# BaguaSys/bagua

Measured on AMD Instinct MI355X. Metric: images/sec (whole node), VGG16 GradientAllReduce vs ByteGrad at 1/2/4/8 MI355X, higher is better.
Workload: dtype bf16; 1 GPU; model=vgg16, algorithm=gradient_allreduce, backend=bagua, global_batch=32, image_size=224, parallelism=dp1

## Files before the change

bagua_amd/models/vgg.py:

```python

from typing import List, Union

import torch
import torch.nn as nn
import torch.nn.functional as F

from ..ops import conv_epilogue

_CFGS = {
    "A": [64, "M", 128, "M", 256, 256, "M", 512, 512, "M", 512, 512, "M"],
    "B": [64, 64, "M", 128, 128, "M", 256, 256, "M", 512, 512, "M",
          512, 512, "M"],
    "D": [64, 64, "M", 128, 128, "M", 256, 256, 256, "M", 512, 512, 512,
          "M", 512, 512, 512, "M"],
    "E": [64, 64, "M", 128, 128, "M", 256, 256, 256, 256, "M",
          512, 512, 512, 512, "M", 512, 512, 512, 512, "M"],
}


class VGG(nn.Module):
    def __init__(self, cfg: List[Union[int, str]], num_classes: int = 1000,
                 batch_norm: bool = False, dropout: float = 0.5):
        super().__init__()
        layers: List[nn.Module] = []
        in_ch = 3
        for v in cfg:
            if v == "M":
                layers.append(nn.MaxPool2d(kernel_size=2, stride=2))
            else:
                layers.append(nn.Conv2d(in_ch, v, kernel_size=3, padding=1))
                if batch_norm:
                    layers.append(nn.BatchNorm2d(v))
                layers.append(nn.ReLU(inplace=True))
                in_ch = v
        self.features = nn.Sequential(*layers)
        self.avgpool = nn.AdaptiveAvgPool2d((7, 7))
        self.classifier = nn.Sequential(
            nn.Linear(512 * 7 * 7, 4096),
            nn.ReLU(True),
            nn.Dropout(p=dropout),
            nn.Linear(4096, 4096),
            nn.ReLU(True),
            nn.Dropout(p=dropout),
            nn.Linear(4096, num_classes),
        )

    torch_bias_grad = False

    def _features(self, x: torch.Tensor) -> torch.Tensor:
        if _has_hooks(self.features):
            return self.features(x)
        mods = list(self.features)
        i = 0
        while i < len(mods):
            m = mods[i]
            step = _fusable(mods, i)
            if step:
                pool = step == 3 and conv_epilogue.conv_eligible(x, m, True)
                if pool or conv_epilogue.conv_eligible(x, m, False):
                    x = F.conv2d(x, m.weight, None, m.stride, m.padding,
                                 m.dilation, m.groups)
                    x = conv_epilogue.conv_bias_relu(
                        x, m.bias, pool, self.torch_bias_grad)
                    i += 3 if pool else 2
                    continue
            x = m(x)
            i += 1
        return x

    def forward(self, x: torch.Tensor) -> torch.Tensor:
        x = self._features(x)
        x = self.avgpool(x)
        x = torch.flatten(x, 1)
        return self.classifier(x)


def _has_hooks(m: nn.Module) -> bool:
    return bool(m._forward_hooks or m._forward_pre_hooks
                or m._backward_hooks or m._backward_pre_hooks)


def _fusable(mods, i) -> int:
    if i + 1 >= len(mods):
        return 0
    conv, relu = mods[i], mods[i + 1]
    if type(conv) is not nn.Conv2d or type(relu) is not nn.ReLU:
        return 0
    if _has_hooks(conv) or _has_hooks(relu):
        return 0
    if i + 2 < len(mods):
        p = mods[i + 2]
        if (type(p) is nn.MaxPool2d and not _has_hooks(p)
                and p.kernel_size in (2, (2, 2)) and p.stride in (2, (2, 2))
                and p.padding in (0, (0, 0)) and p.dilation in (1, (1, 1))
                and not p.ceil_mode and not p.return_indices):
            return 3
    return 2


def vgg11(num_classes=1000, batch_norm=False):
    return VGG(_CFGS["A"], num_classes, batch_norm)


def vgg13(num_classes=1000, batch_norm=False):
    return VGG(_CFGS["B"], num_classes, batch_norm)


def vgg16(num_classes=1000, batch_norm=False):
    return VGG(_CFGS["D"], num_classes, batch_norm)


def vgg19(num_classes=1000, batch_norm=False):
    return VGG(_CFGS["E"], num_classes, batch_norm)
```

bagua_amd/ops/csrc/core.cpp:

```cpp

#include <torch/extension.h>

#include <hip/hip_runtime_api.h>
#include <rccl/rccl.h>

#include <c10/hip/HIPCachingAllocator.h>
#include <c10/hip/HIPStream.h>

#include <chrono>
#include <cmath>
#include <condition_variable>
#include <cstring>
#include <memory>
#include <mutex>
#include <optional>
#include <stdexcept>
#include <string>
#include <thread>
#include <vector>

extern "C" {
void bagua_ew_launch(int op, int dtype, void* x, const void* y, float f,
                     size_t n, hipStream_t stream);
void bagua_async_avg_launch(int dtype, void* x, const void* reduced,
                            const void* x_copy, float nranks, size_t n,
                            hipStream_t stream);
void bagua_reduce_chunk_launch(int dtype, void* x, int num_chunks,
                               int target_chunk, int average, size_t chunk,
                               hipStream_t stream);
void bagua_compress_launch(int dtype, const void* x, uint8_t* out,
                           uint32_t* scratch, uint32_t* partials,
                           size_t chunk, size_t chunk_stride,
                           int num_chunks_total, int chunk_begin,
                           int chunk_count, hipStream_t stream);
void bagua_decompress_launch(int dtype, const uint8_t* in, void* x,
                             size_t chunk, size_t chunk_stride,
                             int chunk_begin, int chunk_count,
                             hipStream_t stream);
void bagua_dequant_reduce_launch(int dtype, const uint8_t* in, void* x,
                                 size_t chunk, size_t chunk_stride,
                                 int num_chunks, int target_chunk,
                                 int average, hipStream_t stream);
void bagua_fused_sgd_launch(float* p, const float* g, float* m, float lr,
                            float momentum, float dampening,
                            float weight_decay, int nesterov,
                            int momentum_initialized, size_t n,
                            hipStream_t stream);
void bagua_fused_adam_launch(float* p, const float* g, float* m, float* v,
                             float lr, float beta1, float beta2,
                             float one_minus_beta1, float one_minus_beta2,
                             float eps, float weight_decay, int adamw,
                             float bc1, float bc2, size_t n,
                             hipStream_t stream);
void bagua_fused_sgd_mixed_launch(void* p, const void* g, float* master,
                                  float* m, float lr, float momentum,
                                  float dampening, float weight_decay,
                                  int nesterov, int momentum_initialized,
                                  size_t n, hipStream_t stream);
void bagua_fused_sgd_segments_launch(float* p, float* m, float lr,
                                     float momentum, float dampening,
                                     float weight_decay, int nesterov,
                                     int momentum_initialized,
                                     const void* const* grads,
                                     const size_t* begins,
                                     const size_t* numels, size_t count,
                                     hipStream_t stream);
void bagua_fused_sgd_mixed_segments_launch(
    void* p, float* master, float* m, float lr, float momentum,
    float dampening, float weight_decay, int nesterov,
    int momentum_initialized, const void* const* grads, const size_t* begins,
    const size_t* numels, size_t count, hipStream_t stream);
void bagua_fused_adam_segments_launch(
    float* p, float* m, float* v, float lr, float beta1, float beta2,
    float one_minus_beta1, float one_minus_beta2, float eps,
    float weight_decay, int adamw, float bc1, float bc2,
    const void* const* grads, const size_t* begins, const size_t* numels,
    size_t count, hipStream_t stream);
}

extern "C" {
size_t bagua_moe_assign_workspace(int S, int E);
void bagua_moe_assign_slots_launch(const int* expert, int S, int E,
                                   int capacity, const int* base, int* hist,
                                   int* slot, int* counts, int* src,
                                   hipStream_t stream);
void bagua_moe_gather_rows_launch(int dtype, const void* x, const int* src,
                                  void* out, const float* w, const int* dest,
                                  int k, int S, size_t R, int M,
                                  hipStream_t stream);
void bagua_moe_combine_rows_launch(int dtype, const void* eo,
                                   const int* dest, void* out,
                                   const float* w, int k, int S, size_t R,
                                   int M, hipStream_t stream);
void bagua_moe_row_dot_launch(int dtype, const void* g, const void* eo,
                              const int* dest, float* gw, int k, int S,
                              size_t R, int M, hipStream_t stream);
}

extern "C" {
size_t bagua_epi_partial_rows(int dtype, size_t work_rows, int C);
void bagua_epi_bias_relu_launch(int dtype, void* x, const void* bias,
                                size_t rows, int C, hipStream_t stream);
void bagua_epi_bias_relu_pool_launch(int dtype, void* x, const void* bias,
                                     void* p, size_t orows, int Wo, int C,
                                     hipStream_t stream);
void bagua_epi_relu_bwd_launch(int dtype, const void* g, const void* y,
                               void* dx, float* partial, void* db,
                               size_t rows, int C, hipStream_t stream);
void bagua_epi_pool_relu_bwd_launch(int dtype, const void* g, const void* y,
                                    void* dx, float* partial, void* db,
                                    size_t orows, int Wo, int C,
                                    hipStream_t stream);
}

#define HIP_CHECK(cmd)                                                    \
  do {                                                                    \
    hipError_t e = (cmd);                                                 \
    if (e != hipSuccess)                                                  \
      throw std::runtime_error(std::string("HIP error: ") +              \
                               hipGetErrorString(e));                     \
  } while (0)

#define NCCL_CHECK(cmd)                                                   \
  do {                                                                    \
    ncclResult_t r = (cmd);                                               \
    if (r != ncclSuccess)                                                 \
      throw std::runtime_error(std::string("RCCL error: ") +             \
                               ncclGetErrorString(r));                    \
  } while (0)

namespace {

ncclDataType_t nccl_dtype(const at::Tensor& t) {
  switch (t.scalar_type()) {
    case at::kFloat: return ncclFloat32;
    case at::kHalf: return ncclFloat16;
    case at::kBFloat16: return ncclBfloat16;
    case at::kByte: return ncclUint8;
    case at::kLong: return ncclInt64;
    case at::kInt: return ncclInt32;
    case at::kDouble: return ncclFloat64;
    default:
      throw std::runtime_error("unsupported dtype for RCCL collective");
  }
}

ncclRedOp_t nccl_op(int op) {
  switch (op) {
    case 0: return ncclSum;
    case 1: return ncclProd;
    case 2: return ncclMin;
    case 3: return ncclMax;
    case 10: return ncclAvg;
    default:
      throw std::runtime_error("ReduceOp not supported by RCCL backend");
  }
}

int kernel_dtype(const at::Tensor& t) {
  switch (t.scalar_type()) {
    case at::kFloat: return 0;
    case at::kHalf: return 1;
    case at::kBFloat16: return 2;
    default:
      throw std::runtime_error("kernel supports f32/f16/bf16 only");
  }
}

hipStream_t current_stream() {
  return c10::hip::getCurrentHIPStream().stream();
}

void check_device_contig(const at::Tensor& t) {
  TORCH_CHECK(t.is_cuda(), "expected a GPU tensor");
  TORCH_CHECK(t.is_contiguous(), "expected a contiguous tensor");
}

}


class Communicator {
 public:
  Communicator(int rank, int nranks, int device, uintptr_t stream,
               const std::string& uid_bytes)
      : rank_(rank), nranks_(nranks), device_(device),
        stream_((hipStream_t)stream) {
    TORCH_CHECK(uid_bytes.size() == sizeof(ncclUniqueId),
                "bad nccl unique id size");
    HIP_CHECK(hipSetDevice(device_));
    ncclUniqueId id;
    std::memcpy(&id, uid_bytes.data(), sizeof(id));
    NCCL_CHECK(ncclCommInitRank(&comm_, nranks_, id, rank_));
  }

  ~Communicator() {
    if (comm_) ncclCommDestroy(comm_);
  }

  int rank() const { return rank_; }
  int nranks() const { return nranks_; }

  void abort() {
    if (comm_) {
      ncclCommAbort(comm_);
      comm_ = nullptr;
    }
  }

  void destroy() {
    if (comm_) {
      ncclCommDestroy(comm_);
      comm_ = nullptr;
    }
  }

  ncclComm_t raw() const { return comm_; }

  void group_start() { NCCL_CHECK(ncclGroupStart()); }
  void group_end() { NCCL_CHECK(ncclGroupEnd()); }

  bool single_() const { return nranks_ == 1; }
  void copy_(at::Tensor& dst, const at::Tensor& src) {
    if (dst.data_ptr() != src.data_ptr())
      HIP_CHECK(hipMemcpyAsync(dst.data_ptr(), src.data_ptr(),
                               src.numel() * src.element_size(),
                               hipMemcpyDeviceToDevice, stream_));
  }

  void allreduce_inplace(at::Tensor t, int op) {
    if (single_()) return;
    check_device_contig(t);
    NCCL_CHECK(ncclAllReduce(t.data_ptr(), t.data_ptr(), t.numel(),
                             nccl_dtype(t), nccl_op(op), comm_, stream_));
  }

  void allreduce(at::Tensor send, at::Tensor recv, int op) {
    if (single_()) { copy_(recv, send); return; }
    check_device_contig(send);
    check_device_contig(recv);
    NCCL_CHECK(ncclAllReduce(send.data_ptr(), recv.data_ptr(), send.numel(),
                             nccl_dtype(send), nccl_op(op), comm_, stream_));
  }

  void reduce_inplace(at::Tensor t, int dst, int op) {
    if (single_()) return;
    check_device_contig(t);
    NCCL_CHECK(ncclReduce(t.data_ptr(), t.data_ptr(), t.numel(),
                          nccl_dtype(t), nccl_op(op), dst, comm_, stream_));
  }

  void broadcast(at::Tensor t, int src) {
    if (single_()) return;
    check_device_contig(t);
    NCCL_CHECK(ncclBroadcast(t.data_ptr(), t.data_ptr(), t.numel(),
                             nccl_dtype(t), src, comm_, stream_));
  }

  void allgather(at::Tensor send, at::Tensor recv) {
    if (single_()) { copy_(recv, send); return; }
    check_device_contig(send);
    check_device_contig(recv);
    TORCH_CHECK(recv.numel() == send.numel() * nranks_,
                "allgather size mismatch");
    NCCL_CHECK(ncclAllGather(send.data_ptr(), recv.data_ptr(), send.numel(),
                             nccl_dtype(send), comm_, stream_));
  }

// ... 841 lines not shown
    check_moe_weights(*w, k, S);
    w_ptr = (const float*)w->data_ptr();
    dest_ptr = (const int*)dest->data_ptr();
  }
  bagua_moe_gather_rows_launch(kernel_dtype(x), x.data_ptr(),
                               (const int*)src.data_ptr(), out.data_ptr(),
                               w_ptr, dest_ptr, (int)k, (int)S,
                               (size_t)src.numel(), (int)x.size(1),
                               current_stream());
}

static void moe_combine_rows(at::Tensor eo, at::Tensor dest, at::Tensor out,
                             std::optional<at::Tensor> w) {
  check_moe_rows(eo, "eo");
  check_moe_rows(out, "out");
  const int64_t k = check_moe_dest(dest);
  const int64_t S = dest.size(1);
  TORCH_CHECK(out.scalar_type() == eo.scalar_type(), "out dtype mismatch");
  TORCH_CHECK(out.size(0) == S && out.size(1) == eo.size(1),
              "out must be (S, M)");
  const float* w_ptr = nullptr;
  if (w.has_value()) {
    check_moe_weights(*w, k, S);
    w_ptr = (const float*)w->data_ptr();
  }
  bagua_moe_combine_rows_launch(kernel_dtype(eo), eo.data_ptr(),
                                (const int*)dest.data_ptr(), out.data_ptr(),
                                w_ptr, (int)k, (int)S, (size_t)eo.size(0),
                                (int)eo.size(1), current_stream());
}

static void moe_row_dot(at::Tensor g, at::Tensor eo, at::Tensor dest,
                        at::Tensor gw) {
  check_moe_rows(g, "g");
  check_moe_rows(eo, "eo");
  const int64_t k = check_moe_dest(dest);
  const int64_t S = dest.size(1);
  TORCH_CHECK(g.scalar_type() == eo.scalar_type(), "g/eo dtype mismatch");
  TORCH_CHECK(g.size(0) == S && g.size(1) == eo.size(1),
              "g must be (S, M)");
  check_moe_weights(gw, k, S);
  bagua_moe_row_dot_launch(kernel_dtype(g), g.data_ptr(), eo.data_ptr(),
                           (const int*)dest.data_ptr(),
                           (float*)gw.data_ptr(), (int)k, (int)S,
                           (size_t)eo.size(0), (int)g.size(1),
                           current_stream());
}


static int64_t check_epi_act(const at::Tensor& t, const char* what) {
  TORCH_CHECK(t.is_cuda(), what, " must be a GPU tensor");
  TORCH_CHECK(t.dim() == 4 &&
                  t.is_contiguous(at::MemoryFormat::ChannelsLast),
              what, " must be 4-d and channels-last contiguous");
  const int64_t vec = 16 / (int64_t)t.element_size();
  const int64_t C = t.size(1);
  TORCH_CHECK(C > 0 && C % vec == 0 && C / vec <= 256, what,
              ": C must be a multiple of ", vec, " and at most ", 256 * vec);
  TORCH_CHECK(((uintptr_t)t.data_ptr() & 15u) == 0, what,
              " must be 16-byte aligned");
  const int64_t rows = t.size(0) * t.size(2) * t.size(3);
  TORCH_CHECK(rows < kInt31, what, ": N*H*W must be below 2^31");
  return rows;
}

static void check_epi_like(const at::Tensor& t, const at::Tensor& ref,
                           const char* what) {
  check_epi_act(t, what);
  TORCH_CHECK(t.sizes() == ref.sizes() &&
                  t.scalar_type() == ref.scalar_type() &&
                  t.device() == ref.device(),
              what, ": shape, dtype or device mismatch");
}

static void check_epi_bias(const at::Tensor& b, const at::Tensor& act,
                           const char* what) {
  check_device_contig(b);
  TORCH_CHECK(b.dim() == 1 && b.size(0) == act.size(1) &&
                  b.scalar_type() == act.scalar_type() &&
                  b.device() == act.device(),
              what, " must be 1-d of C elements, in the activation's dtype "
              "and on its device");
}

static void check_epi_pooled(const at::Tensor& p, const at::Tensor& y,
                             const char* what) {
  TORCH_CHECK(y.size(2) % 2 == 0 && y.size(3) % 2 == 0,
              "pooling needs even H and W");
  check_epi_act(p, what);
  TORCH_CHECK(p.size(0) == y.size(0) && p.size(1) == y.size(1) &&
                  p.size(2) == y.size(2) / 2 && p.size(3) == y.size(3) / 2 &&
                  p.scalar_type() == y.scalar_type() &&
                  p.device() == y.device(),
              what, " must be (N, C, H/2, W/2) in the activation's dtype");
}

static void conv_bias_relu_(at::Tensor x, at::Tensor bias) {
  const int64_t rows = check_epi_act(x, "x");
  check_epi_bias(bias, x, "bias");
  bagua_epi_bias_relu_launch(kernel_dtype(x), x.data_ptr(), bias.data_ptr(),
                             (size_t)rows, (int)x.size(1), current_stream());
}

static void conv_bias_relu_pool_(at::Tensor x, at::Tensor bias,
                                 at::Tensor p) {
  check_epi_act(x, "x");
  check_epi_bias(bias, x, "bias");
  check_epi_pooled(p, x, "p");
  bagua_epi_bias_relu_pool_launch(
      kernel_dtype(x), x.data_ptr(), bias.data_ptr(), p.data_ptr(),
      (size_t)(p.size(0) * p.size(2) * p.size(3)), (int)p.size(3),
      (int)x.size(1), current_stream());
}

static at::Tensor epi_partial(const at::Tensor& y, int64_t work_rows) {
  const int64_t blocks = (int64_t)bagua_epi_partial_rows(
      kernel_dtype(y), (size_t)work_rows, (int)y.size(1));
  return at::empty({blocks, y.size(1)}, y.options().dtype(at::kFloat));
}

static void conv_relu_bwd(at::Tensor g, at::Tensor y, at::Tensor dx,
                          std::optional<at::Tensor> db) {
  const int64_t rows = check_epi_act(y, "y");
  check_epi_like(g, y, "g");
  check_epi_like(dx, y, "dx");
  at::Tensor partial;
  if (db.has_value()) {
    check_epi_bias(*db, y, "db");
    partial = epi_partial(y, rows);
  }
  bagua_epi_relu_bwd_launch(
      kernel_dtype(y), g.data_ptr(), y.data_ptr(), dx.data_ptr(),
      db.has_value() ? (float*)partial.data_ptr() : nullptr,
      db.has_value() ? db->data_ptr() : nullptr, (size_t)rows,
      (int)y.size(1), current_stream());
}

static void conv_pool_relu_bwd(at::Tensor g, at::Tensor y, at::Tensor dx,
                               std::optional<at::Tensor> db) {
  check_epi_act(y, "y");
  check_epi_pooled(g, y, "g");
  check_epi_like(dx, y, "dx");
  const int64_t orows = g.size(0) * g.size(2) * g.size(3);
  at::Tensor partial;
  if (db.has_value()) {
    check_epi_bias(*db, y, "db");
    partial = epi_partial(y, orows);
  }
  bagua_epi_pool_relu_bwd_launch(
      kernel_dtype(y), g.data_ptr(), y.data_ptr(), dx.data_ptr(),
      db.has_value() ? (float*)partial.data_ptr() : nullptr,
      db.has_value() ? db->data_ptr() : nullptr, (size_t)orows,
      (int)g.size(3), (int)y.size(1), current_stream());
}

static py::bytes nccl_unique_id() {
  ncclUniqueId id;
  NCCL_CHECK(ncclGetUniqueId(&id));
  return py::bytes((const char*)&id, sizeof(id));
}



namespace {
ncclDataType_t c_dtype(int d) {
  switch (d) {
    case 0: return ncclFloat32;
    case 1: return ncclFloat16;
    case 2: return ncclBfloat16;
    case 3: return ncclUint8;
    case 4: return ncclInt64;
    default: return ncclFloat32;
  }
}
}

extern "C" {

void* bagua_comm_create(int rank, int nranks, int device,
                        uintptr_t stream, const char* uid_bytes,
                        size_t uid_len) {
  try {
    return new Communicator(rank, nranks, device, stream,
                            std::string(uid_bytes, uid_len));
  } catch (...) {
    return nullptr;
  }
}

void bagua_comm_destroy(void* comm) {
  delete (Communicator*)comm;
}

int bagua_comm_rank(void* comm) { return ((Communicator*)comm)->rank(); }
int bagua_comm_nranks(void* comm) {
  return ((Communicator*)comm)->nranks();
}
void bagua_comm_abort(void* comm) { ((Communicator*)comm)->abort(); }

int bagua_comm_allreduce_inplace(void* comm, void* ptr, size_t numel,
                                 int dtype, int op, uintptr_t stream) {
  Communicator* c = (Communicator*)comm;
  if (c->nranks() == 1) return 0;
  return ncclAllReduce(ptr, ptr, numel, c_dtype(dtype), nccl_op(op),
                       c->raw(), (hipStream_t)stream) == ncclSuccess
             ? 0 : -1;
}

int bagua_comm_broadcast(void* comm, void* ptr, size_t numel, int dtype,
                         int src, uintptr_t stream) {
  Communicator* c = (Communicator*)comm;
  if (c->nranks() == 1) return 0;
  return ncclBroadcast(ptr, ptr, numel, c_dtype(dtype), src, c->raw(),
                       (hipStream_t)stream) == ncclSuccess ? 0 : -1;
}

int bagua_comm_allgather_inplace(void* comm, void* ptr, size_t numel,
                                 int dtype, uintptr_t stream) {
  Communicator* c = (Communicator*)comm;
  if (c->nranks() == 1) return 0;
  size_t chunk = numel / c->nranks();
  size_t es = dtype == 3 ? 1 : (dtype == 1 || dtype == 2) ? 2
              : dtype == 4 ? 8 : 4;
  char* own = (char*)ptr + c->rank() * chunk * es;
  return ncclAllGather(own, ptr, chunk, c_dtype(dtype), c->raw(),
                       (hipStream_t)stream) == ncclSuccess ? 0 : -1;
}

int bagua_nccl_unique_id(char* out, size_t cap) {
  if (cap < sizeof(ncclUniqueId)) return -1;
  ncclUniqueId id;
  if (ncclGetUniqueId(&id) != ncclSuccess) return -1;
  std::memcpy(out, &id, sizeof(id));
  return (int)sizeof(id);
}


static size_t c_esize(int dtype) {
  switch (dtype) {
    case 3: return 1;
    case 1: case 2: return 2;
    case 4: return 8;
    default: return 4;
  }
}

int bagua_comm_reduce_inplace(void* comm, void* ptr, size_t numel,
                              int dtype, int dst, int op,
                              uintptr_t stream) {
  Communicator* c = (Communicator*)comm;
  if (c->nranks() == 1) return 0;
  return ncclReduce(ptr, ptr, numel, c_dtype(dtype), nccl_op(op), dst,
                    c->raw(), (hipStream_t)stream) == ncclSuccess ? 0 : -1;
}

int bagua_comm_reduce_scatter_inplace(void* comm, void* ptr, size_t numel,
                                      int dtype, int op, uintptr_t stream) {
  Communicator* c = (Communicator*)comm;
  if (c->nranks() == 1) return 0;
  if (numel % c->nranks() != 0) return -2;
  size_t chunk = numel / c->nranks();
  char* own = (char*)ptr + c->rank() * chunk * c_esize(dtype);
  return ncclReduceScatter(ptr, own, chunk, c_dtype(dtype), nccl_op(op),
                           c->raw(), (hipStream_t)stream) == ncclSuccess
             ? 0 : -1;
}

int bagua_comm_alltoall(void* comm, const void* send, void* recv,
                        size_t numel, int dtype, uintptr_t stream) {
  Communicator* c = (Communicator*)comm;
  if (c->nranks() == 1) {
    return hipMemcpyAsync(recv, send, numel * c_esize(dtype),
                          hipMemcpyDeviceToDevice,
                          (hipStream_t)stream) == hipSuccess ? 0 : -1;
  }
  if (numel % c->nranks() != 0) return -2;
  return ncclAllToAll(send, recv, numel / c->nranks(), c_dtype(dtype),
                      c->raw(), (hipStream_t)stream) == ncclSuccess
             ? 0 : -1;
}

int bagua_comm_send(void* comm, const void* ptr, size_t numel, int dtype,
                    int dst, uintptr_t stream) {
  Communicator* c = (Communicator*)comm;
  return ncclSend(ptr, numel, c_dtype(dtype), dst, c->raw(),
                  (hipStream_t)stream) == ncclSuccess ? 0 : -1;
}

int bagua_comm_recv(void* comm, void* ptr, size_t numel, int dtype,
                    int src, uintptr_t stream) {
  Communicator* c = (Communicator*)comm;
  return ncclRecv(ptr, numel, c_dtype(dtype), src, c->raw(),
                  (hipStream_t)stream) == ncclSuccess ? 0 : -1;
}

int bagua_comm_gather(void* comm, const void* send, void* recv,
                      size_t numel, int dtype, int dst, uintptr_t stream) {
  Communicator* c = (Communicator*)comm;
  size_t es = c_esize(dtype);
  if (ncclGroupStart() != ncclSuccess) return -1;
  if (c->rank() == dst) {
    for (int r = 0; r < c->nranks(); ++r) {
      if (ncclRecv((char*)recv + (size_t)r * numel * es, numel,
                   c_dtype(dtype), r, c->raw(),
                   (hipStream_t)stream) != ncclSuccess)
        return -1;
    }
  }
  if (ncclSend(send, numel, c_dtype(dtype), dst, c->raw(),
               (hipStream_t)stream) != ncclSuccess)
    return -1;
  return ncclGroupEnd() == ncclSuccess ? 0 : -1;
}

int bagua_comm_scatter(void* comm, const void* send, void* recv,
                       size_t numel, int dtype, int src, uintptr_t stream) {
  Communicator* c = (Communicator*)comm;
  size_t es = c_esize(dtype);
  if (ncclGroupStart() != ncclSuccess) return -1;
  if (c->rank() == src) {
    for (int r = 0; r < c->nranks(); ++r) {
      if (ncclSend((const char*)send + (size_t)r * numel * es, numel,
                   c_dtype(dtype), r, c->raw(),
                   (hipStream_t)stream) != ncclSuccess)
        return -1;
    }
  }
  if (ncclRecv(recv, numel, c_dtype(dtype), src, c->raw(),
               (hipStream_t)stream) != ncclSuccess)
    return -1;
  return ncclGroupEnd() == ncclSuccess ? 0 : -1;
}

int bagua_comm_group_start(void) {
  return ncclGroupStart() == ncclSuccess ? 0 : -1;
}

int bagua_comm_group_end(void) {
  return ncclGroupEnd() == ncclSuccess ? 0 : -1;
}

int bagua_comm_barrier(void* comm, void* scratch_one_elem,
                       uintptr_t stream) {
  Communicator* c = (Communicator*)comm;
  if (c->nranks() > 1) {
    if (ncclAllReduce(scratch_one_elem, scratch_one_elem, 1, ncclFloat32,
                      ncclSum, c->raw(),
                      (hipStream_t)stream) != ncclSuccess)
      return -1;
  }
  return hipStreamSynchronize((hipStream_t)stream) == hipSuccess ? 0 : -1;
}

}

PYBIND11_MODULE(TORCH_EXTENSION_NAME, m) {
  m.doc() = "bagua_amd native core (RCCL over xGMI + CDNA4 kernels)";

  py::class_<Communicator, std::shared_ptr<Communicator>>(m, "Communicator")
      .def(py::init<int, int, int, uintptr_t, const std::string&>())
      .def("rank", &Communicator::rank)
      .def("nranks", &Communicator::nranks)
      .def("abort", &Communicator::abort)
      .def("destroy", &Communicator::destroy)
      .def("group_start", &Communicator::group_start)
      .def("group_end", &Communicator::group_end)
      .def("allreduce_inplace", &Communicator::allreduce_inplace)
      .def("allreduce", &Communicator::allreduce)
      .def("reduce_inplace", &Communicator::reduce_inplace)
      .def("broadcast", &Communicator::broadcast)
      .def("allgather", &Communicator::allgather)
      .def("allgather_inplace", &Communicator::allgather_inplace)
      .def("reduce_scatter", &Communicator::reduce_scatter)
      .def("reduce_scatter_inplace", &Communicator::reduce_scatter_inplace)
      .def("alltoall", &Communicator::alltoall)
      .def("alltoall_inplace", &Communicator::alltoall_inplace)
      .def("alltoall_v", &Communicator::alltoall_v)
      .def("send", &Communicator::send)
      .def("recv", &Communicator::recv)
      .def("gather", &Communicator::gather)
      .def("gather_inplace", &Communicator::gather_inplace)
      .def("scatter", &Communicator::scatter)
      .def("scatter_inplace", &Communicator::scatter_inplace);

  py::class_<BucketExecutor>(m, "BucketExecutor")
      .def(py::init<std::shared_ptr<Communicator>,
                    std::shared_ptr<Communicator>,
                    std::shared_ptr<Communicator>, uintptr_t>(),
           py::arg("global_comm"), py::arg("intra_comm") = nullptr,
           py::arg("inter_comm") = nullptr, py::arg("stream") = 0)
      .def("register_bucket", &BucketExecutor::register_bucket)
      .def("execute", &BucketExecutor::execute)
      .def("wait_pending", &BucketExecutor::wait_pending)
      .def("synchronize", &BucketExecutor::synchronize)
      .def("clear_buckets", &BucketExecutor::clear_buckets);

  py::class_<P2PAlltoAll>(m, "P2PAlltoAll")
      .def(py::init<int, int, uintptr_t, int64_t>(), py::arg("rank"),
           py::arg("nranks"), py::arg("stream"), py::arg("capacity"))
      .def("handles", &P2PAlltoAll::handles)
      .def("connect", &P2PAlltoAll::connect)
      .def("capacity", &P2PAlltoAll::capacity)
      .def("alltoall", &P2PAlltoAll::alltoall)
      .def("allgather_inplace", &P2PAlltoAll::allgather_inplace);

  m.def("nccl_unique_id", &nccl_unique_id);
  m.def("average_inplace", &average_inplace);
  m.def("add_inplace", &add_inplace);
  m.def("substract_inplace", &substract_inplace);
  m.def("addmul_inplace", &addmul_inplace);
  m.def("divide_inplace", &divide_inplace);
  m.def("async_model_average", &async_model_average);
  m.def("reduce_chunk_inplace", &reduce_chunk_inplace);
  m.def("compress_chunked", &compress_chunked);
  m.def("decompress_chunked", &decompress_chunked);
  m.def("dequant_reduce", &dequant_reduce);
  m.def("compressed_chunk_stride", &compressed_chunk_stride);
  m.def("fused_sgd_step", &fused_sgd_step);
  m.def("fused_sgd_mixed_step", &fused_sgd_mixed_step);
  m.def("fused_adam_step", &fused_adam_step);
  m.def("fused_sgd_step_segments", &fused_sgd_step_segments, py::arg("p"),
        py::arg("grads"), py::arg("offsets"), py::arg("m"), py::arg("lr"),
        py::arg("momentum"), py::arg("dampening"), py::arg("weight_decay"),
        py::arg("nesterov"), py::arg("momentum_initialized"));
  m.def("fused_sgd_mixed_step_segments", &fused_sgd_mixed_step_segments,
        py::arg("p"), py::arg("grads"), py::arg("offsets"),
        py::arg("master"), py::arg("m"), py::arg("lr"), py::arg("momentum"),
        py::arg("dampening"), py::arg("weight_decay"), py::arg("nesterov"),
        py::arg("momentum_initialized"));
  m.def("fused_adam_step_segments", &fused_adam_step_segments, py::arg("p"),
        py::arg("grads"), py::arg("offsets"), py::arg("m"), py::arg("v"),
        py::arg("step"), py::arg("lr"), py::arg("beta1"), py::arg("beta2"),
        py::arg("eps"), py::arg("weight_decay"), py::arg("adamw"));
  m.def("moe_assign_slots", &moe_assign_slots, py::arg("expert"),
        py::arg("num_experts"), py::arg("capacity"), py::arg("base"),
        py::arg("slot"), py::arg("counts"), py::arg("src"));
  m.def("moe_gather_rows", &moe_gather_rows, py::arg("x"), py::arg("src"),
        py::arg("out"), py::arg("w") = py::none(),
        py::arg("dest") = py::none());
  m.def("moe_combine_rows", &moe_combine_rows, py::arg("eo"),
        py::arg("dest"), py::arg("out"), py::arg("w") = py::none());
  m.def("moe_row_dot", &moe_row_dot);
  m.def("conv_bias_relu_", &conv_bias_relu_, py::arg("x"), py::arg("bias"));
  m.def("conv_bias_relu_pool_", &conv_bias_relu_pool_, py::arg("x"),
        py::arg("bias"), py::arg("p"));
  m.def("conv_relu_bwd", &conv_relu_bwd, py::arg("g"), py::arg("y"),
        py::arg("dx"), py::arg("db") = py::none());
  m.def("conv_pool_relu_bwd", &conv_pool_relu_bwd, py::arg("g"),
        py::arg("y"), py::arg("dx"), py::arg("db") = py::none());
}
```

setup.py:

```python

import os

from setuptools import find_packages, setup

os.environ.setdefault("PYTORCH_ROCM_ARCH", "gfx950")

from torch.utils import cpp_extension

ROCM_HOME = os.environ.get("ROCM_HOME", "/opt/rocm")

ext = cpp_extension.CUDAExtension(
    name="bagua_amd._C",
    sources=[
        "bagua_amd/ops/csrc/core.cpp",
        "bagua_amd/ops/csrc/kernels.hip",
        "bagua_amd/ops/csrc/moe_kernels.hip",
        "bagua_amd/ops/csrc/epilogue_kernels.hip",
    ],
    include_dirs=[os.path.join(ROCM_HOME, "include")],
    libraries=["rccl"],
    library_dirs=[os.path.join(ROCM_HOME, "lib")],
    extra_compile_args={
        "cxx": ["-O3", "-std=c++17"],
        "nvcc": ["-O3", "-std=c++17"],
    },
)

setup(
    name="bagua_amd",
    version="0.1.0",
    packages=find_packages(include=["bagua_amd", "bagua_amd.*"]),
    ext_modules=[ext],
    cmdclass={"build_ext": cpp_extension.BuildExtension},
    entry_points={
        "console_scripts": [
            "baguarun = bagua_amd.distributed.baguarun:main",
            "bagua_sys_perf = bagua_amd.distributed.sys_perf:main",
        ],
    },
)
```

Before: 4343 images/s.

## Add fused MFMA kernel for VGG first conv with bias and ReLU

Adds a dedicated HIP kernel for the 3-to-64-channel 3x3 first convolution. The forward pass does an implicit GEMM with MFMA and fuses bias and ReLU. The backward pass fuses the ReLU mask with the weight and bias gradient reduction, then runs a separate finalize kernel. The goal is to replace MIOpen's poorly suited small-Cin convolution and its separate epilogue and bias-grad passes. It only applies to bf16 channels-last inputs that do not require grad, so no input gradient is computed. The path may not trigger if the input is not channels-last.

```diff
diff --git a/bagua_amd/models/vgg.py b/bagua_amd/models/vgg.py
--- a/bagua_amd/models/vgg.py
+++ b/bagua_amd/models/vgg.py
@@ -5,7 +5,7 @@
 import torch.nn as nn
 import torch.nn.functional as F
 
-from ..ops import conv_epilogue
+from ..ops import conv_epilogue, first_conv
 
 _CFGS = {
     "A": [64, "M", 128, "M", 256, 256, "M", 512, 512, "M", 512, 512, "M"],
@@ -55,6 +55,11 @@
         while i < len(mods):
             m = mods[i]
             step = _fusable(mods, i)
+            if (step == 2 and not self.torch_bias_grad
+                    and first_conv.eligible(x, m)):
+                x = first_conv.first_conv_bias_relu(x, m.weight, m.bias)
+                i += 2
+                continue
             if step:
                 pool = step == 3 and conv_epilogue.conv_eligible(x, m, True)
                 if pool or conv_epilogue.conv_eligible(x, m, False):
diff --git a/bagua_amd/ops/csrc/core.cpp b/bagua_amd/ops/csrc/core.cpp
--- a/bagua_amd/ops/csrc/core.cpp
+++ b/bagua_amd/ops/csrc/core.cpp
@@ -17,6 +17,7 @@
 #include <stdexcept>
 #include <string>
 #include <thread>
+#include <tuple>
 #include <vector>
 
 extern "C" {
@@ -113,6 +114,19 @@
                                     hipStream_t stream);
 }
 
+extern "C" {
+size_t bagua_first_conv_partial_rows(int N, int H, int W);
+size_t bagua_first_conv_partial_cols();
+void bagua_first_conv_fwd_launch(const void* x, const void* w,
+                                 const long* wstride, const void* bias,
+                                 void* y, int N, int H, int W,
+                                 hipStream_t stream);
+void bagua_first_conv_bwd_launch(const void* g, const void* y, const void* x,
+                                 float* partial, void* dw,
+                                 const long* wstride, void* db, int N, int H,
+                                 int W, hipStream_t stream);
+}
+
 #define HIP_CHECK(cmd)                                                    \
   do {                                                                    \
     hipError_t e = (cmd);                                                 \
@@ -1260,6 +1274,81 @@
       db.has_value() ? (float*)partial.data_ptr() : nullptr,
       db.has_value() ? db->data_ptr() : nullptr, (size_t)orows,
       (int)g.size(3), (int)y.size(1), current_stream());
+}
+
+
+static int64_t check_first_conv_x(const at::Tensor& x) {
+  TORCH_CHECK(x.is_cuda(), "x must be a GPU tensor");
+  TORCH_CHECK(x.scalar_type() == at::kBFloat16, "x must be bf16");
+  TORCH_CHECK(x.dim() == 4 && x.size(1) == 3 &&
+                  x.is_contiguous(at::MemoryFormat::ChannelsLast),
+              "x must be (N, 3, H, W) and channels-last contiguous");
+  const int64_t rows = x.size(0) * x.size(2) * x.size(3);
+  TORCH_CHECK(rows > 0 && rows < kInt31,
+              "x: N*H*W must be at least 1 and below 2^31");
+  return rows;
+}
+
+static void check_first_conv_weight(const at::Tensor& w,
+                                    const at::Tensor& x, const char* what) {
+  TORCH_CHECK(w.is_cuda() && w.device() == x.device() &&
+                  w.scalar_type() == at::kBFloat16,
+              what, " must be bf16 on x's device");
+  TORCH_CHECK(w.dim() == 4 && w.size(0) == 64 && w.size(1) == 3 &&
+                  w.size(2) == 3 && w.size(3) == 3,
+              what, " must be (64, 3, 3, 3)");
+  TORCH_CHECK(w.is_contiguous() ||
+                  w.is_contiguous(at::MemoryFormat::ChannelsLast),
+              what, " must be contiguous or channels-last contiguous");
+}
+
+static void check_first_conv_act(const at::Tensor& t, const at::Tensor& x,
+                                 const char* what) {
+  check_epi_act(t, what);
+  TORCH_CHECK(t.scalar_type() == at::kBFloat16 && t.device() == x.device() &&
+                  t.size(0) == x.size(0) && t.size(1) == 64 &&
+                  t.size(2) == x.size(2) && t.size(3) == x.size(3),
+              what, " must be (N, 64, H, W) bf16 on x's device");
+}
+
+static at::Tensor first_conv_bias_relu(at::Tensor x, at::Tensor weight,
+                                       at::Tensor bias) {
+  check_first_conv_x(x);
+  check_first_conv_weight(weight, x, "weight");
+  at::Tensor y = at::empty({x.size(0), 64, x.size(2), x.size(3)},
+                           x.options().memory_format(
+                               at::MemoryFormat::ChannelsLast));
+  check_first_conv_act(y, x, "y");
+  check_epi_bias(bias, y, "bias");
+  const long ws[4] = {(long)weight.stride(0), (long)weight.stride(1),
+                      (long)weight.stride(2), (long)weight.stride(3)};
+  bagua_first_conv_fwd_launch(x.data_ptr(), weight.data_ptr(), ws,
+                              bias.data_ptr(), y.data_ptr(), (int)x.size(0),
+                              (int)x.size(2), (int)x.size(3),
+                              current_stream());
+  return y;
+}
+
+static std::tuple<at::Tensor, at::Tensor> first_conv_bias_relu_bwd(
+    at::Tensor g, at::Tensor y, at::Tensor x, at::Tensor weight_like) {
+  check_first_conv_x(x);
+  check_first_conv_weight(weight_like, x, "weight_like");
+  check_first_conv_act(y, x, "y");
+  check_first_conv_act(g, x, "g");
+  at::Tensor dw = at::empty_strided(weight_like.sizes(),
+                                    weight_like.strides(), y.options());
+  at::Tensor db = at::empty({64}, y.options());
+  const int N = (int)x.size(0), H = (int)x.size(2), W = (int)x.size(3);
+  at::Tensor partial = at::empty(
+      {(int64_t)bagua_first_conv_partial_rows(N, H, W),
+       (int64_t)bagua_first_conv_partial_cols()},
+      y.options().dtype(at::kFloat));
+  const long ws[4] = {(long)dw.stride(0), (long)dw.stride(1),
+                      (long)dw.stride(2), (long)dw.stride(3)};
+  bagua_first_conv_bwd_launch(g.data_ptr(), y.data_ptr(), x.data_ptr(),
+                              (float*)partial.data_ptr(), dw.data_ptr(), ws,
+                              db.data_ptr(), N, H, W, current_stream());
+  return std::make_tuple(dw, db);
 }
 
 static py::bytes nccl_unique_id() {
@@ -1556,4 +1645,8 @@
         py::arg("dx"), py::arg("db") = py::none());
   m.def("conv_pool_relu_bwd", &conv_pool_relu_bwd, py::arg("g"),
         py::arg("y"), py::arg("dx"), py::arg("db") = py::none());
-}
+  m.def("first_conv_bias_relu", &first_conv_bias_relu, py::arg("x"),
+        py::arg("weight"), py::arg("bias"));
+  m.def("first_conv_bias_relu_bwd", &first_conv_bias_relu_bwd, py::arg("g"),
+        py::arg("y"), py::arg("x"), py::arg("weight_like"));
+}
diff --git a/bagua_amd/ops/csrc/first_conv_kernels.hip b/bagua_amd/ops/csrc/first_conv_kernels.hip
--- /dev/null
+++ b/bagua_amd/ops/csrc/first_conv_kernels.hip
@@ -0,0 +1,412 @@
+
+#include <hip/hip_runtime.h>
+#include <cstdint>
+
+#define FC_BLOCK 256
+#define FC_WAVES (FC_BLOCK / 64)
+#define FC_TW 32
+#define FC_TH FC_WAVES
+#define FC_CIN 3
+#define FC_COUT 64
+#define FC_K 27
+#define FC_KB 28
+#define FC_XROW ((FC_TW + 2) * FC_CIN)
+#define FC_XTILE ((FC_TH + 2) * FC_XROW)
+#define FC_XLOADS ((FC_XTILE + FC_BLOCK - 1) / FC_BLOCK)
+#define FC_VEC_PER_ROW (FC_TW * FC_COUT / 8)
+#define FC_FIN_OUT 8
+#define FC_FIN_SL (FC_BLOCK / FC_FIN_OUT)
+
+static_assert(FC_VEC_PER_ROW == FC_BLOCK, "one 16-byte vector per thread and "
+                                          "tile row");
+static_assert((FC_COUT * FC_KB) % FC_FIN_OUT == 0, "finalize grid");
+
+namespace {
+
+typedef __bf16 bf16x8 __attribute__((ext_vector_type(8)));
+typedef float f32x16 __attribute__((ext_vector_type(16)));
+
+union Frag {
+  bf16x8 v;
+  uint16_t e[8];
+  uint4 q;
+};
+
+__device__ __forceinline__ float bf16_to_f(uint16_t b) {
+  return __uint_as_float((uint32_t)b << 16);
+}
+
+__device__ __forceinline__ uint16_t f_to_bf16(float v) {
+  if (v != v) return 0x7FC0;
+  const uint32_t u = __float_as_uint(v);
+  return (uint16_t)((u + ((u >> 16) & 1u) + 0x7FFFu) >> 16);
+}
+
+__device__ __forceinline__ uint16_t bias_relu(uint16_t x, float b) {
+  const uint16_t t = f_to_bf16(bf16_to_f(x) + b);
+  const float f = bf16_to_f(t);
+  return (f != f) ? t : (uint16_t)(__float_as_uint(fmaxf(f, 0.f)) >> 16);
+}
+
+struct Geom {
+  int H, W, tiles_x, tiles_y, ntiles;
+};
+
+struct TilePos {
+  int n, y0, x0;
+};
+
+__device__ __forceinline__ TilePos tile_pos(int t, const Geom& g) {
+  TilePos p;
+  const int tx = t % g.tiles_x;
+  const int q = t / g.tiles_x;
+  const int ty = q % g.tiles_y;
+  p.n = q / g.tiles_y;
+  p.y0 = ty * FC_TH;
+  p.x0 = tx * FC_TW;
+  return p;
+}
+
+__device__ __forceinline__ void load_x_tile(const uint16_t* __restrict__ x,
+                                            const Geom& g, const TilePos& p,
+                                            uint16_t (&xr)[FC_XLOADS]) {
+#pragma unroll
+  for (int u = 0; u < FC_XLOADS; ++u) {
+    const int e = (int)threadIdx.x + u * FC_BLOCK;
+    xr[u] = 0;
+    if (e < FC_XTILE) {
+      const int ty = e / FC_XROW;
+      const int rem = e - ty * FC_XROW;
+      const int tx = rem / FC_CIN;
+      const int gy = p.y0 - 1 + ty, gx = p.x0 - 1 + tx;
+      if (gy >= 0 && gy < g.H && gx >= 0 && gx < g.W) {
+        const size_t pix = ((size_t)p.n * g.H + gy) * g.W + gx;
+        xr[u] = x[pix * FC_CIN + (rem - tx * FC_CIN)];
+      }
+    }
+  }
+}
+
+__device__ __forceinline__ void store_x_tile(uint16_t* xt,
+                                             const uint16_t (&xr)[FC_XLOADS]) {
+#pragma unroll
+  for (int u = 0; u < FC_XLOADS; ++u) {
+    const int e = (int)threadIdx.x + u * FC_BLOCK;
+    if (e < FC_XTILE) xt[e] = xr[u];
+  }
+}
+
+__device__ __forceinline__ int patch_off(int k) {
+  const int ky = k / 9;
+  return ky * FC_XROW + (k - ky * 9);
+}
+
+
+__global__ void __launch_bounds__(FC_BLOCK)
+first_conv_fwd_kernel(const uint16_t* __restrict__ x,
+                      const uint16_t* __restrict__ w, long ws0, long ws1,
+                      long ws2, long ws3, const uint16_t* __restrict__ bias,
+                      uint4* __restrict__ y, Geom g) {
+  __shared__ uint16_t xt[FC_XTILE];
+  __shared__ uint4 yt[FC_TH * FC_VEC_PER_ROW];
+
+  const int lane = threadIdx.x & 63, wave = threadIdx.x >> 6;
+  const int r = lane & 31, h = lane >> 5;
+
+  const int rc = (r & 0x13) | ((r & 4) << 1) | ((r & 8) >> 1);
+  Frag a[2][2];
+#pragma unroll
+  for (int s = 0; s < 2; ++s) {
+#pragma unroll
+    for (int j = 0; j < 8; ++j) {
+      const int k = 16 * s + 8 * h + j;
+      const bool in = k < FC_K;
+      const int ky = k / 9, kx = (k / 3) % 3, ci = k % 3;
+#pragma unroll
+      for (int mt = 0; mt < 2; ++mt) {
+        const long co = 32 * mt + rc;
+        a[mt][s].e[j] =
+            in ? w[co * ws0 + ci * ws1 + ky * ws2 + kx * ws3] : (uint16_t)0;
+      }
+    }
+  }
+  Frag b[4];
+#pragma unroll
+  for (int t = 0; t < 4; ++t) {
+#pragma unroll
+    for (int q = 0; q < 8; ++q)
+      b[t].e[q] = bias[32 * (t >> 1) + 16 * (t & 1) + 8 * h + q];
+  }
+
+  uint16_t xr[FC_XLOADS];
+  int t = blockIdx.x;
+  if (t < g.ntiles) load_x_tile(x, g, tile_pos(t, g), xr);
+  for (; t < g.ntiles; t += gridDim.x) {
+    const TilePos p = tile_pos(t, g);
+    __syncthreads();
+    store_x_tile(xt, xr);
+    __syncthreads();
+    if (t + (int)gridDim.x < g.ntiles)
+      load_x_tile(x, g, tile_pos(t + gridDim.x, g), xr);
+
+    const uint16_t* px = xt + wave * FC_XROW + r * FC_CIN;
+    f32x16 acc[2];
+#pragma unroll
+    for (int mt = 0; mt < 2; ++mt) {
+#pragma unroll
+      for (int i = 0; i < 16; ++i) acc[mt][i] = 0.f;
+    }
+#pragma unroll
+    for (int s = 0; s < 2; ++s) {
+      Frag bf;
+#pragma unroll
+      for (int j = 0; j < 8; ++j) {
+        const int k0 = 16 * s + j, k1 = k0 + 8;
+        const int off = h ? (k1 < FC_K ? patch_off(k1) : 0) : patch_off(k0);
+        const uint16_t v = px[off];
+        bf.e[j] = (k1 < FC_K || !h) ? v : (uint16_t)0;
+      }
+#pragma unroll
+      for (int mt = 0; mt < 2; ++mt)
+        acc[mt] = __builtin_amdgcn_mfma_f32_32x32x16_bf16(a[mt][s].v, bf.v,
+                                                          acc[mt], 0, 0, 0);
+    }
+
+    uint4* yw = yt + wave * FC_VEC_PER_ROW;
+#pragma unroll
+    for (int tq = 0; tq < 4; ++tq) {
+      Frag o;
+#pragma unroll
+      for (int q = 0; q < 8; ++q)
+        o.e[q] = bias_relu(f_to_bf16(acc[tq >> 1][8 * (tq & 1) + q]),
+                           bf16_to_f(b[tq].e[q]));
+      const int chunk = 4 * (tq >> 1) + 2 * (tq & 1) + h;
+      yw[r * 8 + (chunk ^ (r & 7))] = o.q;
+    }
+    __syncthreads();
+    const int gy = p.y0 + wave;
+    if (gy < g.H) {
+      uint4* yrow = y + (((size_t)p.n * g.H + gy) * g.W + p.x0) * (FC_COUT / 8);
+#pragma unroll
+      for (int i = 0; i < 4; ++i) {
+        const int v = i * 64 + lane;
+        const int pr = v >> 3, chunk = v & 7;
+        if (p.x0 + pr < g.W) yrow[v] = yw[pr * 8 + (chunk ^ (pr & 7))];
+      }
+    }
+  }
+}
+
+
+__device__ __forceinline__ void load_gy_tile(const uint4* __restrict__ gv,
+                                             const uint4* __restrict__ yv,
+                                             const Geom& g, const TilePos& p,
+                                             uint4 (&gr)[FC_TH],
+                                             uint4 (&yr)[FC_TH]) {
+  const int pr = threadIdx.x >> 3;
+#pragma unroll
+  for (int u = 0; u < FC_TH; ++u) {
+    gr[u] = make_uint4(0, 0, 0, 0);
+    yr[u] = make_uint4(0, 0, 0, 0);
+    const int gy = p.y0 + u;
+    if (gy < g.H && p.x0 + pr < g.W) {
+      const size_t v = (((size_t)p.n * g.H + gy) * g.W + p.x0) * (FC_COUT / 8)
+                       + threadIdx.x;
+      gr[u] = gv[v];
+      yr[u] = yv[v];
+    }
+  }
+}
+
+__device__ __forceinline__ uint32_t relu_mask2(uint32_t g, uint32_t y) {
+  const float ylo = __uint_as_float(y << 16);
+  const float yhi = __uint_as_float(y & 0xFFFF0000u);
+  uint32_t m = 0xFFFFFFFFu;
+  if (ylo <= 0.f) m &= 0xFFFF0000u;
+  if (yhi <= 0.f) m &= 0x0000FFFFu;
+  return g & m;
+}
+
+__global__ void __launch_bounds__(FC_BLOCK)
+first_conv_bwd_kernel(const uint4* __restrict__ gv,
+                      const uint4* __restrict__ yv,
+                      const uint16_t* __restrict__ x,
+                      float* __restrict__ partial, Geom g) {
+  __shared__ uint16_t xt[FC_XTILE];
+  __shared__ uint4 dxt[FC_TH * FC_VEC_PER_ROW];
+  static_assert(sizeof(dxt) >= 2 * 16 * 64 * sizeof(float), "reduce buffer");
+
+  const int lane = threadIdx.x & 63, wave = threadIdx.x >> 6;
+  const int r = lane & 31, h = lane >> 5;
+
+  const int lo = (int)((long)blockIdx.x * g.ntiles / gridDim.x);
+  const int hi = (int)((long)(blockIdx.x + 1) * g.ntiles / gridDim.x);
+
+  const int coff = r < FC_K ? patch_off(r) : 0;
+  const uint16_t bconst = r == FC_K ? (uint16_t)0x3F80 : (uint16_t)0;
+
+  f32x16 acc[2];
+#pragma unroll
+  for (int mt = 0; mt < 2; ++mt) {
+#pragma unroll
+    for (int i = 0; i < 16; ++i) acc[mt][i] = 0.f;
+  }
+
+  uint4 gr[FC_TH], yr[FC_TH];
+  uint16_t xr[FC_XLOADS];
+  if (lo < hi) {
+    const TilePos p = tile_pos(lo, g);
+    load_gy_tile(gv, yv, g, p, gr, yr);
+    load_x_tile(x, g, p, xr);
+  }
+  for (int t = lo; t < hi; ++t) {
+    const TilePos pc = tile_pos(t, g);
+    const int wlim = pc.y0 + wave < g.H ? g.W - pc.x0 : 0;
+    __syncthreads();
+#pragma unroll
+    for (int u = 0; u < FC_TH; ++u) {
+      uint4 d;
+      d.x = relu_mask2(gr[u].x, yr[u].x);
+      d.y = relu_mask2(gr[u].y, yr[u].y);
+      d.z = relu_mask2(gr[u].z, yr[u].z);
+      d.w = relu_mask2(gr[u].w, yr[u].w);
+      dxt[u * FC_VEC_PER_ROW + threadIdx.x] = d;
+    }
+    store_x_tile(xt, xr);
+    __syncthreads();
+    if (t + 1 < hi) {
+      const TilePos p = tile_pos(t + 1, g);
+      load_gy_tile(gv, yv, g, p, gr, yr);
+      load_x_tile(x, g, p, xr);
+    }
+
+    const uint16_t* dxe = reinterpret_cast<const uint16_t*>(dxt) +
+                          wave * FC_TW * FC_COUT;
+    const uint16_t* px = xt + wave * FC_XROW + coff;
+#pragma unroll
+    for (int ks = 0; ks < 2; ++ks) {
+      Frag bf, af[2];
+#pragma unroll
+      for (int j = 0; j < 8; ++j) {
+        const int pix = 16 * ks + 8 * h + j;
+        const uint16_t bv = r < FC_K ? px[pix * FC_CIN] : bconst;
+        bf.e[j] = pix < wlim ? bv : (uint16_t)0;
+#pragma unroll
+        for (int mt = 0; mt < 2; ++mt)
+          af[mt].e[j] = dxe[pix * FC_COUT + 32 * mt + r];
+      }
+#pragma unroll
+      for (int mt = 0; mt < 2; ++mt)
+        acc[mt] = __builtin_amdgcn_mfma_f32_32x32x16_bf16(af[mt].v, bf.v,
+                                                          acc[mt], 0, 0, 0);
+    }
+  }
+
+  float* red = reinterpret_cast<float*>(dxt);
+  for (int wv = 0; wv < FC_WAVES; ++wv) {
+    __syncthreads();
+    if (wave == wv) {
+#pragma unroll
+      for (int mt = 0; mt < 2; ++mt) {
+#pragma unroll
+        for (int i = 0; i < 16; ++i) {
+          const int idx = (mt * 16 + i) * 64 + lane;
+          red[idx] = wv == 0 ? acc[mt][i] : red[idx] + acc[mt][i];
+        }
+      }
+    }
+  }
+  __syncthreads();
+  float* out = partial + (size_t)blockIdx.x * (FC_COUT * FC_KB);
+  for (int idx = threadIdx.x; idx < 2 * 16 * 64; idx += FC_BLOCK) {
+    const int mt = idx >> 10, i = (idx >> 6) & 15, ln = idx & 63;
+    const int col = ln & 31;
+    const int row = (i & 3) + 8 * (i >> 2) + 4 * (ln >> 5);
+    if (col < FC_KB) out[(32 * mt + row) * FC_KB + col] = red[idx];
+  }
+}
+
+__global__ void __launch_bounds__(FC_BLOCK)
+first_conv_bwd_finalize_kernel(const float* __restrict__ partial, int nrows,
+                               uint16_t* __restrict__ dw, long ws0, long ws1,
+                               long ws2, long ws3, uint16_t* __restrict__ db) {
+  __shared__ float red[FC_FIN_SL][FC_FIN_OUT];
+  const int cl = threadIdx.x % FC_FIN_OUT, sl = threadIdx.x / FC_FIN_OUT;
+  const int o = blockIdx.x * FC_FIN_OUT + cl;
+  float s = 0.f;
+#pragma unroll 8
+  for (int b = sl; b < nrows; b += FC_FIN_SL)
+    s += partial[(size_t)b * (FC_COUT * FC_KB) + o];
+  red[sl][cl] = s;
+  __syncthreads();
+  if (sl == 0) {
+    float t = 0.f;
+#pragma unroll
+    for (int k = 0; k < FC_FIN_SL; ++k) t += red[k][cl];
+    const long co = o / FC_KB;
+    const int k = o - (int)co * FC_KB;
+    if (k == FC_K) {
+      db[co] = f_to_bf16(t);
+    } else {
+      const int ky = k / 9, kx = (k / 3) % 3, ci = k % 3;
+      dw[co * ws0 + ci * ws1 + ky * ws2 + kx * ws3] = f_to_bf16(t);
+    }
+  }
+}
+
+inline Geom geom_of(int N, int H, int W) {
+  Geom g;
+  g.H = H;
+  g.W = W;
+  g.tiles_x = (W + FC_TW - 1) / FC_TW;
+  g.tiles_y = (H + FC_TH - 1) / FC_TH;
+  g.ntiles = N * g.tiles_y * g.tiles_x;
+  return g;
+}
+
+#define FC_FWD_MAX_GRID 512
+#define FC_BWD_MAX_GRID 768
+
+inline unsigned grid_of(const Geom& g, int cap) {
+  return (unsigned)(g.ntiles < cap ? g.ntiles : cap);
+}
+
+}
+
+
+extern "C" {
+
+size_t bagua_first_conv_partial_rows(int N, int H, int W) {
+  return grid_of(geom_of(N, H, W), FC_BWD_MAX_GRID);
+}
+
+size_t bagua_first_conv_partial_cols() { return FC_COUT * FC_KB; }
+
+void bagua_first_conv_fwd_launch(const void* x, const void* w,
+                                 const long* wstride, const void* bias,
+                                 void* y, int N, int H, int W,
+                                 hipStream_t stream) {
+  const Geom g = geom_of(N, H, W);
+  hipLaunchKernelGGL(first_conv_fwd_kernel, dim3(grid_of(g, FC_FWD_MAX_GRID)), dim3(FC_BLOCK), 0,
+                     stream, (const uint16_t*)x, (const uint16_t*)w,
+                     wstride[0], wstride[1], wstride[2], wstride[3],
+                     (const uint16_t*)bias, (uint4*)y, g);
+}
+
+void bagua_first_conv_bwd_launch(const void* g, const void* y, const void* x,
+                                 float* partial, void* dw,
+                                 const long* wstride, void* db, int N, int H,
+                                 int W, hipStream_t stream) {
+  const Geom gm = geom_of(N, H, W);
+  const unsigned grid = grid_of(gm, FC_BWD_MAX_GRID);
+  hipLaunchKernelGGL(first_conv_bwd_kernel, dim3(grid), dim3(FC_BLOCK), 0,
+                     stream, (const uint4*)g, (const uint4*)y,
+                     (const uint16_t*)x, partial, gm);
+  hipLaunchKernelGGL(first_conv_bwd_finalize_kernel,
+                     dim3(FC_COUT * FC_KB / FC_FIN_OUT), dim3(FC_BLOCK), 0,
+                     stream, (const float*)partial, (int)grid,
+                     (uint16_t*)dw, wstride[0], wstride[1], wstride[2],
+                     wstride[3], (uint16_t*)db);
+}
+
+}
diff --git a/bagua_amd/ops/first_conv.py b/bagua_amd/ops/first_conv.py
--- /dev/null
+++ b/bagua_amd/ops/first_conv.py
@@ -0,0 +1,80 @@
+
+import torch
+from torch import Tensor
+from torch.autograd.function import once_differentiable
+
+from . import native
+
+IN_CHANNELS = 3
+OUT_CHANNELS = 64
+
+
+def _dense_weight(w: Tensor) -> bool:
+    return w.is_contiguous() \
+        or w.is_contiguous(memory_format=torch.channels_last)
+
+
+def eligible(x: Tensor, conv: torch.nn.Conv2d) -> bool:
+    if not x.is_cuda or x.dim() != 4 or x.requires_grad:
+        return False
+    if torch.is_autocast_enabled():
+        return False
+    w, b = conv.weight, conv.bias
+    if b is None:
+        return False
+    if not (x.dtype == w.dtype == b.dtype == torch.bfloat16):
+        return False
+    if (conv.in_channels != IN_CHANNELS or conv.out_channels != OUT_CHANNELS
+            or x.shape[1] != IN_CHANNELS
+            or tuple(conv.kernel_size) != (3, 3)
+            or tuple(conv.stride) != (1, 1)
+            or isinstance(conv.padding, str)
+            or tuple(conv.padding) != (1, 1)
+            or tuple(conv.dilation) != (1, 1) or conv.groups != 1
+            or conv.padding_mode != "zeros"):
+        return False
+    n, _, h, wd = x.shape
+    if n < 1 or h < 1 or wd < 1 or n * h * wd >= 2 ** 31:
+        return False
+    if not x.is_contiguous(memory_format=torch.channels_last):
+        return False
+    if x.data_ptr() % 16 != 0:
+        return False
+    if not _dense_weight(w) or not b.is_contiguous():
+        return False
+    native.require()
+    return True
+
+
+def _channels_last(t: Tensor) -> Tensor:
+    t = t.contiguous(memory_format=torch.channels_last)
+    if t.data_ptr() % 16 != 0:
+        t = t.clone(memory_format=torch.channels_last)
+    return t
+
+
+class _FirstConvBiasRelu(torch.autograd.Function):
+
+    @staticmethod
+    def forward(ctx, x, weight, bias):
+        ctx.set_materialize_grads(False)
+        y = native.require().first_conv_bias_relu(x, weight.detach(),
+                                                  bias.detach())
+        ctx.save_for_backward(x, y, weight)
+        return y
+
+    @staticmethod
+    @once_differentiable
+    def backward(ctx, g):
+        if g is None or not (ctx.needs_input_grad[1]
+                             or ctx.needs_input_grad[2]):
+            return None, None, None
+        x, y, weight = ctx.saved_tensors
+        dw, db = native.require().first_conv_bias_relu_bwd(
+            _channels_last(g), y, x, weight)
+        return (None, dw if ctx.needs_input_grad[1] else None,
+                db if ctx.needs_input_grad[2] else None)
+
+
+def first_conv_bias_relu(x: Tensor, weight: Tensor, bias: Tensor) -> Tensor:
+    return _FirstConvBiasRelu.apply(x, weight, bias)
diff --git a/setup.py b/setup.py
--- a/setup.py
+++ b/setup.py
@@ -16,6 +16,7 @@
         "bagua_amd/ops/csrc/kernels.hip",
         "bagua_amd/ops/csrc/moe_kernels.hip",
         "bagua_amd/ops/csrc/epilogue_kernels.hip",
+        "bagua_amd/ops/csrc/first_conv_kernels.hip",
     ],
     include_dirs=[os.path.join(ROCM_HOME, "include")],
     libraries=["rccl"],
```

After: 4467 images/s, median of 6. 2.9% higher.
